# orybkin/video-gcp

Measured on AMD Instinct MI355X. Metric: predicted frames/sec, 64x64x3 seq_len=80 gcp_tree (posterior forward + all loss terms, model(inputs) and model.loss() of train.py:157-159, batch-stat BatchNorm), higher is better.
Workload: dtype f32 (encoder / decoder convs and the tree GEMMs from 512 rows: split-f16 MFMA with f32 accumulate, f32-equivalent; everything else exact f32 MFMA)

## Files before the change

### video-gcp_amd/csrc/conv3x3_lowres.hip

```cpp
#include "common.h"
#include "split_mfma.h"

namespace {

template <int CT, int HIN, int NCHUNK, int FPU>
struct LowresCfg {
    static constexpr int NW = 3 * CT, NT = NW * 64;
    static constexpr int NPIX = HIN * HIN, UPIX = FPU * NPIX, NPG = UPIX / 16, WOUT = 2 * HIN, HOUT = 2 * HIN;
    static constexpr int COUT = CT * 16, CIN = NCHUNK * 32, C4 = COUT / 4, Q4 = CIN / 4;
    static constexpr int YS = COUT + 4;
    static constexpr int PLANE_BYTES = UPIX * 64;
    static constexpr int PLANES_BYTES = NCHUNK * 2 * PLANE_BYTES;
    static constexpr int Y_BYTES = 9 * UPIX * YS * 4;
    static constexpr int Z_BYTES = FPU * 3 * HIN * WOUT * COUT * 4;
    static constexpr int PZ_BYTES = PLANES_BYTES > Z_BYTES ? PLANES_BYTES : Z_BYTES;
    static constexpr int TAB_BYTES = (2 * CIN + COUT) * 4;
    static constexpr int STAT_BYTES = NT * 8 * 4;
    static constexpr int LDS_BYTES = PZ_BYTES + Y_BYTES + 64 + TAB_BYTES + STAT_BYTES;
    static constexpr int NSLOT = UPIX * Q4;
    static constexpr int NS = (NSLOT + NT - 1) / NT;
    static constexpr int NHZ = FPU * 3 * HIN * WOUT * C4;
    static constexpr int NOUT = FPU * HOUT * WOUT * C4;
    static constexpr int NO = (NOUT + NT - 1) / NT;
    static_assert(NT % C4 == 0 && NT % Q4 == 0, "a thread keeps one channel quad of the input and one of the output");
    static_assert(NOUT * 16 <= Y_BYTES, "the finished output waits in the Y buffer");
    static_assert(LDS_BYTES <= 160 * 1024, "LDS");
};

__device__ __forceinline__ void up_taps(const int h, const int n, int& s0, int& s1, float& w0, float& w1) {
    const int s = h >> 1;
    const bool odd = h & 1;
    s0 = odd ? s : max(s - 1, 0);
    s1 = odd ? min(s + 1, n - 1) : s;
    w0 = odd ? 0.75f : 0.25f;
    w1 = 1.f - w0;
}

template <int CT, int HIN, int NCHUNK, int FPU>
__global__ void __launch_bounds__(3 * CT * 64, 1) conv3x3_lowres_kernel(const gcpx_conv_args a, const int stat_rows) {
    using Cfg = LowresCfg<CT, HIN, NCHUNK, FPU>;
    constexpr int NT = Cfg::NT, NPIX = Cfg::NPIX, UPIX = Cfg::UPIX, NPG = Cfg::NPG, WOUT = Cfg::WOUT, HOUT = Cfg::HOUT, COUT = Cfg::COUT;
    constexpr int C4 = Cfg::C4, Q4 = Cfg::Q4, NS = Cfg::NS, NSLOT = Cfg::NSLOT, NO = Cfg::NO, NOUT = Cfg::NOUT, NHZ = Cfg::NHZ;
    constexpr int PLANE = Cfg::PLANE_BYTES, YS = Cfg::YS, FS = HOUT * WOUT * COUT;
    extern __shared__ float4 smem4[];
    char* planes = reinterpret_cast<char*>(smem4);
    float* Z = reinterpret_cast<float*>(smem4);
    float* Y = reinterpret_cast<float*>(planes + Cfg::PZ_BYTES);
    unsigned* smax = reinterpret_cast<unsigned*>(planes + Cfg::PZ_BYTES + Cfg::Y_BYTES);
    float* bnS = reinterpret_cast<float*>(smax + 16);
    float* bnT = bnS + Cfg::CIN;
    float* biasT = bnT + Cfg::CIN;
    float4* stat = reinterpret_cast<float4*>(biasT + COUT);

    const int tid = threadIdx.x, lane = tid & 63;
    const int wave = __builtin_amdgcn_readfirstlane(tid >> 6);
    const int j = lane & 15, q = lane >> 4;
    const int tx = wave % 3, ct = wave / 3;
    const int F = a.F;
    const int ew = a.w_split_log2_dev ? __builtin_amdgcn_readfirstlane(*a.w_split_log2_dev) : a.w_split_log2;

    h8 wreg[3][NCHUNK][2];
    {
        const char* wbase = reinterpret_cast<const char*>(a.wpk_split) + lane * 16;
#pragma unroll
        for (int ty = 0; ty < 3; ++ty)
#pragma unroll
            for (int ch = 0; ch < NCHUNK; ++ch) {
                const char* wp = wbase + (size_t)(((ch * 9 + ty * 3 + tx) * CT + ct) * 2048);
                wreg[ty][ch][0] = *reinterpret_cast<const h8*>(wp);
                wreg[ty][ch][1] = *reinterpret_cast<const h8*>(wp + 1024);
            }
    }
    if (tid < NCHUNK) smax[tid] = 0u;

    const int cgq = (tid % Q4) * 4, chq = cgq >> 5;
    const int c0 = a.src[0].C;
    const bool first = cgq < c0;
    const int clq = first ? cgq : cgq - c0;
    const float* sptr = (first ? a.src[0].ptr : a.src[1].ptr) + clq;
    const int srcC = first ? a.src[0].C : a.src[1].C;
    const int fdiv = first ? a.src[0].frame_div : a.src[1].frame_div;
    const float slope = (first ? a.src[0].act : a.src[1].act) == GCPX_ACT_LRELU ? 0.2f : 1.f;
    const int c4q = tid % C4;
    for (int c = tid; c < Cfg::CIN; c += NT) {
        const gcpx_conv_src& sr = c < c0 ? a.src[0] : a.src[1];
        const int cl = c < c0 ? c : c - c0;
        bnS[c] = sr.scale ? sr.scale[cl] : 1.f;
        bnT[c] = sr.scale ? sr.shift[cl] : 0.f;
    }
    if (tid < COUT) biasT[tid] = a.bias[tid];
    stat[tid * 2] = stat[tid * 2 + 1] = make_float4(0.f, 0.f, 0.f, 0.f);

    float4 pre[NS];
    auto issue_loads = [&](const int f0, const int t) {
#pragma unroll
        for (int k = 0; k < NS; ++k) {
            const int idx = t + NT * k;
            pre[k] = make_float4(0.f, 0.f, 0.f, 0.f);
            if (NSLOT % NT == 0 || idx < NSLOT) {
                const int up = idx / Q4;
                const int f = min(f0 + up / NPIX, F - 1);
                pre[k] = *reinterpret_cast<const float4*>(sptr + ((size_t)(f / fdiv) * NPIX + up % NPIX) * srcC);
            }
        }
    };
    float4* O = reinterpret_cast<float4*>(Y);
    int pf0 = -1;
    auto store_out = [&](const int t) __attribute__((always_inline)) {
        float* outu = a.out + (size_t)pf0 * FS;
#pragma unroll
        for (int k = 0; k < NO; ++k) {
            const int i = t + NT * k;
            if ((NOUT % NT == 0 || i < NOUT) && pf0 + i / (HOUT * WOUT * C4) < F) *reinterpret_cast<float4*>(outu + i * 4) = O[i];
        }
    };

    const int nunits = (F + FPU - 1) / FPU;
    int u = blockIdx.x;
    if (u < nunits) issue_loads(u * FPU, tid);
    __syncthreads();

    for (; u < nunits; u += gridDim.x) {
        const int f0 = u * FPU;
        int tl = tid;
        asm volatile("" : "+v"(tl));
        float4 v[NS];
        float m = 0.f;
        const float4 bn_s = *reinterpret_cast<const float4*>(bnS + cgq), bn_t = *reinterpret_cast<const float4*>(bnT + cgq);
#pragma unroll
        for (int k = 0; k < NS; ++k) {
            float4 t = pre[k];
            t.x = fmaf(t.x, bn_s.x, bn_t.x); t.y = fmaf(t.y, bn_s.y, bn_t.y); t.z = fmaf(t.z, bn_s.z, bn_t.z); t.w = fmaf(t.w, bn_s.w, bn_t.w);
            t.x = t.x > 0.f ? t.x : t.x * slope; t.y = t.y > 0.f ? t.y : t.y * slope;
            t.z = t.z > 0.f ? t.z : t.z * slope; t.w = t.w > 0.f ? t.w : t.w * slope;
            if (!(NSLOT % NT == 0 || tl + NT * k < NSLOT)) t = make_float4(0.f, 0.f, 0.f, 0.f);
            v[k] = t;
            m = fmaxf(m, fmaxf(fmaxf(fabsf(t.x), fabsf(t.y)), fmaxf(fabsf(t.z), fabsf(t.w))));
        }
        m = fmaxf(m, __shfl_xor(m, 1));
        m = fmaxf(m, __shfl_xor(m, 2));
        m = fmaxf(m, __shfl_xor(m, 4));
        if ((lane & 7) == 0) atomicMax(&smax[chq], __float_as_uint(m));
        if (pf0 >= 0) store_out(tl);
        __syncthreads();
        int exr[NCHUNK];
#pragma unroll
        for (int ch = 0; ch < NCHUNK; ++ch) {
            const float amax = __uint_as_float(smax[ch]);
            int ec = 14 + 127 - (int)((__float_as_uint(amax) >> 23) & 0xff);
            ec = __builtin_amdgcn_readfirstlane(amax > 0.f ? max(-100, min(min(100, 126 - ew), ec)) : min(100, 126 - ew));
            exr[ch] = ch == 0 ? ec : min(ec, exr[ch - 1]);
        }
        {
            int ex = exr[0];
#pragma unroll
            for (int c = 1; c < NCHUNK; ++c) ex = chq == c ? exr[c] : ex;
            const float sc = __uint_as_float((unsigned)(127 + ex) << 23);
#pragma unroll
            for (int k = 0; k < NS; ++k) {
                const int idx = tl + NT * k;
                if (NSLOT % NT == 0 || idx < NSLOT) {
                    float4 s = v[k];
                    s.x *= sc; s.y *= sc; s.z *= sc; s.w *= sc;
                    h4 p1, p2;
                    p1[0] = (_Float16)s.x; p1[1] = (_Float16)s.y; p1[2] = (_Float16)s.z; p1[3] = (_Float16)s.w;
                    p2[0] = (_Float16)(s.x - (float)p1[0]); p2[1] = (_Float16)(s.y - (float)p1[1]);
                    p2[2] = (_Float16)(s.z - (float)p1[2]); p2[3] = (_Float16)(s.w - (float)p1[3]);
                    char* dst = planes + chq * 2 * PLANE + (idx / Q4) * 64 + (cgq & 31) * 2;
                    *reinterpret_cast<h4*>(dst) = p1;
                    *reinterpret_cast<h4*>(dst + PLANE) = p2;
                }
            }
        }
        __syncthreads();
        if (tid < NCHUNK) smax[tid] = 0u;
        if (u + (int)gridDim.x < nunits) issue_loads((u + gridDim.x) * FPU, tl);

        f32x4 acc[3][NPG];
#pragma unroll
        for (int ty = 0; ty < 3; ++ty)
#pragma unroll
            for (int pg = 0; pg < NPG; ++pg) acc[ty][pg] = f32x4{0, 0, 0, 0};
        __builtin_amdgcn_s_setprio(1);
#pragma unroll
        for (int ch = 0; ch < NCHUNK; ++ch) {
            if (ch > 0 && exr[ch] != exr[ch - 1]) {
                const float r = __uint_as_float((unsigned)(127 + exr[ch] - exr[ch - 1]) << 23);
#pragma unroll
                for (int ty = 0; ty < 3; ++ty)
#pragma unroll
                    for (int pg = 0; pg < NPG; ++pg) acc[ty][pg] *= r;
            }
#pragma unroll
            for (int pg = 0; pg < NPG; ++pg) {
                const char* bp = planes + ch * 2 * PLANE + (pg * 16 + (tl & 15)) * 64 + ((tl >> 4) & 3) * 16;
                const h8 b1 = *reinterpret_cast<const h8*>(bp);
                const h8 b2 = *reinterpret_cast<const h8*>(bp + PLANE);
#pragma unroll
                for (int ty = 0; ty < 3; ++ty) acc[ty][pg] = mfma32h(wreg[ty][ch][1], b1, acc[ty][pg]);
#pragma unroll
                for (int ty = 0; ty < 3; ++ty) acc[ty][pg] = mfma32h(wreg[ty][ch][0], b2, acc[ty][pg]);
#pragma unroll
                for (int ty = 0; ty < 3; ++ty) acc[ty][pg] = mfma32h(wreg[ty][ch][0], b1, acc[ty][pg]);
            }
        }
        __builtin_amdgcn_s_setprio(0);
        {
            const float inv = __uint_as_float((unsigned)(127 - exr[NCHUNK - 1] - ew) << 23);
#pragma unroll
            for (int ty = 0; ty < 3; ++ty)
#pragma unroll
                for (int pg = 0; pg < NPG; ++pg) {
                    const f32x4 y = acc[ty][pg] * inv;
                    *reinterpret_cast<float4*>(Y + ((ty * 3 + tx) * UPIX + pg * 16 + (tl & 15)) * YS + ct * 16 + ((tl >> 4) & 3) * 4) = make_float4(y[0], y[1], y[2], y[3]);
                }
        }
        __syncthreads();
        int tv = tid;
        asm volatile("" : "+v"(tv));
        float4 ab[NO];
#pragma unroll
        for (int k = 0; k < NO; ++k) ab[k] = *reinterpret_cast<const float4*>(biasT + c4q * 4);
        if (a.addend) {
#pragma unroll
            for (int k = 0; k < NO; ++k) {
                const int i = tv + NT * k;
                if (NOUT % NT == 0 || i < NOUT) {
                    const int f = min(f0 + i / (HOUT * WOUT * C4), F - 1);
                    const float4 ad = *reinterpret_cast<const float4*>(a.addend + (size_t)(f / a.addend_frame_div) * FS + (i % (HOUT * WOUT * C4)) * 4);
                    ab[k].x += ad.x; ab[k].y += ad.y; ab[k].z += ad.z; ab[k].w += ad.w;
                }
            }
        }

#pragma unroll 1
        for (int i = tv; i < NHZ; i += NT) {
            int t = i / C4;
            const int px = t % WOUT; t /= WOUT;
            const int sy = t % HIN; t /= HIN;
            const int ty = t % 3, fl = t / 3;
            float4 z = make_float4(0.f, 0.f, 0.f, 0.f);
#pragma unroll
            for (int kx = 0; kx < 3; ++kx) {
                const int hx = px + kx - 1;
                if (hx >= 0 && hx < WOUT) {
                    int s0, s1; float w0, w1;
                    up_taps(hx, HIN, s0, s1, w0, w1);
                    const float* yp = Y + ((ty * 3 + kx) * UPIX + fl * NPIX + sy * HIN) * YS + c4q * 4;
                    const float4 A = *reinterpret_cast<const float4*>(yp + s0 * YS);
                    const float4 B = *reinterpret_cast<const float4*>(yp + s1 * YS);
                    z.x += w0 * A.x + w1 * B.x; z.y += w0 * A.y + w1 * B.y; z.z += w0 * A.z + w1 * B.z; z.w += w0 * A.w + w1 * B.w;
                }
            }
            *reinterpret_cast<float4*>(Z + i * 4) = z;
        }
        __syncthreads();

        f32x4 st1 = f32x4{0, 0, 0, 0}, st2 = f32x4{0, 0, 0, 0};
#pragma unroll
        for (int k = 0; k < NO; ++k) {
            const int i = tv + NT * k;
            __builtin_amdgcn_sched_barrier(0);
            if (NOUT % NT == 0 || i < NOUT) {
                int t = i / C4;
                const int px = t % WOUT; t /= WOUT;
                const int py = t % HOUT, fl = t / HOUT;
                float4 o = make_float4(0.f, 0.f, 0.f, 0.f);
#pragma unroll
                for (int ky = 0; ky < 3; ++ky) {
                    const int hy = py + ky - 1;
                    if (hy >= 0 && hy < HOUT) {
                        int s0, s1; float w0, w1;
                        up_taps(hy, HIN, s0, s1, w0, w1);
                        const float* zp = Z + (((fl * 3 + ky) * HIN) * WOUT + px) * COUT + c4q * 4;
                        const float4 A = *reinterpret_cast<const float4*>(zp + s0 * WOUT * COUT);
                        const float4 B = *reinterpret_cast<const float4*>(zp + s1 * WOUT * COUT);
                        o.x += w0 * A.x + w1 * B.x; o.y += w0 * A.y + w1 * B.y; o.z += w0 * A.z + w1 * B.z; o.w += w0 * A.w + w1 * B.w;
                    }
                }
                const f32x4 r = f32x4{o.x + ab[k].x, o.y + ab[k].y, o.z + ab[k].z, o.w + ab[k].w};
                O[i] = make_float4(r[0], r[1], r[2], r[3]);
                if (f0 + fl < F) {
                    st1 += r;
                    st2 += r * r;
                }
            }
        }
        {
            const float4 s1 = stat[tid * 2], s2 = stat[tid * 2 + 1];
            stat[tid * 2] = make_float4(s1.x + st1[0], s1.y + st1[1], s1.z + st1[2], s1.w + st1[3]);
            stat[tid * 2 + 1] = make_float4(s2.x + st2[0], s2.y + st2[1], s2.z + st2[2], s2.w + st2[3]);
        }
        pf0 = f0;
    }
    if (pf0 >= 0) store_out(tid);

    if (a.stats_partial) {
        __syncthreads();
        const float* red = reinterpret_cast<const float*>(stat);
        if (tid < 2 * COUT) {
            const int which = tid / COUT, c = tid % COUT;
            float sum = 0.f;
#pragma unroll 4
            for (int m = 0; m < NT / C4; ++m) sum += red[((c >> 2) + C4 * m) * 8 + which * 4 + (c & 3)];
            a.stats_partial[((size_t)blockIdx.x * 2 + which) * COUT + c] = sum;
            for (int r = blockIdx.x + gridDim.x; r < stat_rows; r += gridDim.x) a.stats_partial[((size_t)r * 2 + which) * COUT + c] = 0.f;
        }
    }
}

template <int CT, int HIN, int NCHUNK, int FPU>
int launch_lowres(const gcpx_conv_args* a, hipStream_t stream, int rows) {
    using Cfg = LowresCfg<CT, HIN, NCHUNK, FPU>;
    auto kern = conv3x3_lowres_kernel<CT, HIN, NCHUNK, FPU>;
    static bool attr_set = false;
    if (!attr_set) {
        hipError_t e = hipFuncSetAttribute(reinterpret_cast<const void*>(kern), hipFuncAttributeMaxDynamicSharedMemorySize, Cfg::LDS_BYTES);
        if (e != hipSuccess) {
            gcpx_set_error("conv3x3 lowres: hipFuncSetAttribute(%d B LDS): %s", Cfg::LDS_BYTES, hipGetErrorString(e));
            return GCPX_ERR_HIP;
        }
        attr_set = true;
    }
    const int nunits = (a->F + FPU - 1) / FPU;
    int grid = gcpx_conv_grid() / 2;
    if (a->stats_partial && grid > rows) grid = rows;
    if (grid > nunits) grid = nunits;
    hipLaunchKernelGGL(kern, dim3(grid), dim3(Cfg::NT), Cfg::LDS_BYTES, stream, *a, rows);
    GCPX_CHECK_LAUNCH();
    return GCPX_OK;
}

int lowres_variant(const gcpx_conv_args* a) {
    if (!a || !a->upsample || !a->wpk_split || !a->out || !a->bias) return -1;
    if (a->split_layout != GCPX_SPLIT_PLAIN && a->split_layout != GCPX_SPLIT_LOWRES) return -1;
    if (a->head_mode != GCPX_HEAD_RAW || a->out_act != GCPX_ACT_NONE || a->out_pitch != a->Cout) return -1;
    if (a->src_row_map || a->raw_row_map || a->bwd_r) return -1;
    if (a->Hin != a->Win || a->Hout != 2 * a->Hin || a->Wout != 2 * a->Win || a->F <= 0) return -1;
    if (a->nsrc != 1 && a->nsrc != 2) return -1;
    int cin = 0;
    for (int s = 0; s < a->nsrc; ++s) {
        if (!a->src[s].ptr || a->src[s].C <= 0 || a->src[s].C % 16 || a->src[s].frame_div <= 0) return -1;
        cin += a->src[s].C;
    }
    if (cin != a->Cin) return -1;
    if (a->addend && a->addend_frame_div <= 0) return -1;
    if (a->Cout == 64 && a->Hin == 4 && a->Cin == 128) return 0;
    if (a->Cout == 32 && a->Hin == 8 && a->Cin == 64) return 1;
    if (a->Cout == 32 && a->Hin == 8 && a->Cin == 128) return 2;
    if (a->Cout == 32 && a->Hin == 4 && a->Cin == 128) return 3;
    return -1;
}

}

extern "C" int gcpx_conv3x3_lowres_supported(const gcpx_conv_args* a) { return lowres_variant(a) >= 0 ? 1 : 0; }

int gcpx_launch_lowres(const gcpx_conv_args* a, hipStream_t stream, int rows) {
    switch (lowres_variant(a)) {
        case 0: return launch_lowres<4, 4, 4, 2>(a, stream, rows);
        case 1: return launch_lowres<2, 8, 2, 1>(a, stream, rows);
        case 2: return launch_lowres<2, 8, 4, 1>(a, stream, rows);
        case 3: return launch_lowres<2, 4, 4, 2>(a, stream, rows);
    }
    gcpx_set_error("conv3x3 lowres: GCPX_SPLIT_LOWRES on a problem gcpx_conv3x3_lowres_supported refuses (up=%d Cin=%d Cout=%d Hin=%d)",
                   a->upsample, a->Cin, a->Cout, a->Hin);
    return GCPX_ERR_UNSUPPORTED;
}
```

### video-gcp_amd/weights.py

```python
import ctypes as C
import os
from contextlib import contextmanager

import torch

from . import packing as pk
from . import runtime as rt
from .hparams import GCPHParams
from .params import init_params, encoder_layers, encoder_skip_layers, decoder_layers
from .plan_ops import _addr


class WeightsMixin:

    def _flatten_params(self, params):
        off, self._poff = 0, {}
        for k, v in params.items():
            self._poff[k] = (off, tuple(v.shape))
            off += (v.numel() + 3) // 4 * 4
        self.theta = torch.zeros(off, dtype=torch.float32, device=self.device)
        self.sd = {}
        for k, v in params.items():
            o, shp = self._poff[k]
            view = self.theta[o:o + v.numel()].view(shp)
            view.copy_(v)
            self.sd[k] = view

    def _pack_predictor(self, prefix, out_dim):
        sd = self._psd
        mid = sd[f"{prefix}.input.linear.weight"].shape[0]
        n_mid = 0
        while f"{prefix}.pyramid-{n_mid}.linear.weight" in sd:
            n_mid += 1
        out_pad = (out_dim + 15) // 16 * 16
        w_in = sd[f"{prefix}.input.linear.weight"]
        k_raw = w_in.shape[1]
        if k_raw % 16:
            w_in = torch.cat([w_in, torch.zeros((mid, -k_raw % 16), dtype=w_in.dtype, device=w_in.device)], 1)
        d = dict(mid=mid, n_mid=n_mid, out_dim=out_dim, in_dim=w_in.shape[1], in_dim_raw=k_raw)
        d["w_in"] = pk.pack_gemm(w_in)
        d["b_in"] = sd[f"{prefix}.input.linear.bias"].contiguous()
        if n_mid:
            d["w_mid"] = torch.stack([pk.pack_gemm(sd[f"{prefix}.pyramid-{i}.linear.weight"]) for i in range(n_mid)]).contiguous()
            d["b_mid"] = torch.stack([sd[f"{prefix}.pyramid-{i}.linear.bias"] for i in range(n_mid)]).contiguous()
            d["gn_g"] = torch.stack([sd[f"{prefix}.pyramid-{i}.norm.weight"] for i in range(n_mid)]).contiguous()
            d["gn_b"] = torch.stack([sd[f"{prefix}.pyramid-{i}.norm.bias"] for i in range(n_mid)]).contiguous()
        d["w_out"] = pk.pack_gemm(sd[f"{prefix}.head.linear.weight"])
        d["b_out"] = pk.pad_vec(sd[f"{prefix}.head.linear.bias"], out_pad)
        return d

    def _pack_all(self):
        if self._arena is not None:
            self.repack()
            return
        self.pk = self._pack_tree(self.sd)
        if self._hp.tree_lstm:
            self._pack_fused_embed()
        self._pack_split()
        self._pack_gemm_split()

    def _pack_split(self):
        self.pk_split = {}
        hp = self._hp
        todo = []
        if hp.decoder_distribution == "discrete_logistic_mixture":
            todo.append(("dec.head", "decoder.gen_head.conv.weight", pk.dlm_channel_perm(hp.n_mixtures)))
            if self.head32 and hp.n_mixtures == 10 and hp.head_channels == 100:
                todo.append(("dec.head32", "decoder.gen_head.conv.weight", ("head32", pk.dlm_channel_perm(hp.n_mixtures))))
        hoist16 = set()
        for name, c_prev, c_skip, skip_idx, cout in decoder_layers(hp):
            if cout == 16 and c_prev + c_skip == 32:
                todo.append((f"dec.{name}", f"decoder.net.{name}.conv.weight", "rowfold"))
                if self.split_f16 and skip_idx >= 0 and c_prev == 16 and c_skip == 16 and os.environ.get("GCPX_NO_SKIP_HOIST") is None:
                    hoist16.add(f"dec.{name}")
            elif cout == 16:
                todo.append((f"dec.{name}", f"decoder.net.{name}.conv.weight", None))
            elif cout in (32, 64) and (c_prev + c_skip) % 32 == 0:
                todo.append((f"dec.{name}", f"decoder.net.{name}.conv.weight", "tiled32"))
        for name, cin, cout, norm in self._enc_layers[1:]:
            if cin == 16 or cin % 32 == 0:
                todo.append((f"enc.{name}", f"encoder.net.{name}.conv.weight", "enc4x4"))
        for name, key, perm in todo:
            off, shp = self._poff[key]
            d = {}
            if perm == "enc4x4":
                idx = pk.conv4x4_split_index(shp, off).to(self.device)
            elif perm == "rowfold":
                d["fold"] = torch.zeros(24 * shp[0] * shp[1], dtype=torch.float32, device=self.device)
                d["fold_src"] = (off, shp[0], shp[1])
                idx = pk.conv3x3_fold_index().to(self.device)
            elif perm == "tiled32":
                idx = pk.conv3x3_split32_index(shp, off).to(self.device)
            elif isinstance(perm, tuple) and perm[0] == "head32":
                idx = pk.head32_index(shp, off, perm[1]).to(self.device)
            else:
                idx = pk.conv3x3_split_index(shp, off, perm).to(self.device)
            d.update(idx=idx, out=torch.zeros(2 * idx.numel(), dtype=torch.int16, device=self.device),
                     log2=torch.zeros(1, dtype=torch.int32, device=self.device))
            self.pk_split[name] = d
            if perm == "rowfold" and name in hoist16:
                for tag, cbase in (("f16a", 0), ("f16b", 16)):
                    i16 = pk.conv3x3_fold16_index(shp[1], cbase).to(self.device)
                    self.pk_split[f"{name}.{tag}"] = dict(fold=d["fold"], fold16=True, idx=i16,
                                                          out=torch.zeros(2 * i16.numel(), dtype=torch.int16, device=self.device),
                                                          log2=torch.zeros(1, dtype=torch.int32, device=self.device))
        self.repack_split()

    def repack_split(self, stream=None):
        st = stream if stream is not None else torch.cuda.current_stream(self.device).cuda_stream
        if not self.pk_split:
            return
        tab = self._split_tab
        key = (self.theta.data_ptr(),) + tuple((d["out"].data_ptr(), d["idx"].data_ptr()) for d in self.pk_split.values())
        if tab is None or tab[2] != key:
            descs = []
            for name, d in self.pk_split.items():
                src = d["fold"] if "fold" in d else self.theta
                e = rt.SplitPackDesc()
                e.src, e.idx, e.out, e.log2_out, e.n = src.data_ptr(), d["idx"].data_ptr(), d["out"].data_ptr(), d["log2"].data_ptr(), d["idx"].numel()
                descs.append(e)
            arr = (rt.SplitPackDesc * len(descs))(*descs)
            dev = torch.frombuffer(bytearray(bytes(arr)), dtype=torch.uint8).to(self.device)
            tab = self._split_tab = (dev, len(descs), key, torch.zeros(len(descs), dtype=torch.int32, device=self.device))
        for name, d in self.pk_split.items():
            if "fold_src" in d:
                off, cout, cin = d["fold_src"]
                rt.check(self.lib.gcpx_fold_upsample_weights(self.theta.data_ptr() + 4 * off, cout, cin, d["fold"].data_ptr(), st), "fold_upsample_weights")
        rt.check(self.lib.gcpx_split_pack_group2(tab[0].data_ptr(), tab[1], tab[3].data_ptr(), st), "split_pack_group2")

    def _pack_gemm_split(self):
        self._gsplit = {}
        self._merge_side_rows = int(os.environ.get("GCPX_MERGE_SIDE_ROWS", "512")) or (1 << 60)
        pr = int(os.environ.get("GCPX_GEMM_PLANES_ROWS", "512"))
        self._planes_min_rows = pr if pr > 0 else 1 << 60
        if not self.split_f16:
            return
        for name, W in self.pk.items():
            if not (isinstance(W, dict) and name.startswith("tree")):
                continue
            for key, wpk in W.items():
                if not (key.endswith(".w") and (key.startswith("lstm") or key == "proj.w")):
                    continue
                stack = wpk if wpk.dim() == 5 else wpk[None]
                if (stack.shape[2] * 16) % 64 or (stack.shape[1] * 16) % 64:
                    continue
                packs = [pk.pack_gemm_split(pk.unpack_gemm(w, w.shape[1] * 16)) for w in stack]
                ws = torch.stack([p_[0] for p_ in packs]).contiguous().to(self.device)
                es = torch.tensor([p_[1] for p_ in packs], dtype=torch.int32, device=self.device)
                self._gsplit[wpk.data_ptr()] = (ws, es)

    def _set_split(self, a, name):
        d = self.pk_split.get(name)
        layout = None
        if name == "dec.head" and self.head32 and a.head_mode in (rt.HEAD_DLM_MEAN, rt.HEAD_DLM_NLL, rt.HEAD_DLM_NLL_GRAD) \
                and "dec.head32" in self.pk_split:
            d, layout = self.pk_split["dec.head32"], rt.SPLIT_HEAD32
        if self.split_f16 and d is not None:
            a.wpk_split, a.w_split_log2_dev = d["out"].data_ptr(), d["log2"].data_ptr()
            if layout is None:
                layout = rt.SPLIT_ROWFOLD16 if d.get("fold16") else (rt.SPLIT_ROWFOLD if "fold" in d else rt.SPLIT_PLAIN)
            a.split_layout = layout
            if layout == rt.SPLIT_PLAIN and os.environ.get("GCPX_NO_LOWRES") is None and \
                    (a.Cout == 64 or a.F <= self.lib.gcpx_conv_grid() // 2) and self.lib.gcpx_conv3x3_lowres_supported(C.byref(a)):
                a.split_layout = rt.SPLIT_LOWRES

    def _pack_fused_embed(self):
        hp = self._hp
        for l in range(hp.hierarchy_levels if hp.untied_layers else 1):
            p = f"tree_module.tree_modules.{l}.subgoal_pred"
            sd = self.sd
            We, be = sd[f"{p}.embed.weight"].double(), sd[f"{p}.embed.bias"].double()
            Wih = sd[f"{p}.lstm.0.weight_ih"].double()
            Wf = (Wih @ We).float()
            bf = (Wih @ be).float() + sd[f"{p}.lstm.0.bias_ih"]
            w, b = pk.lstm_gate_interleave(Wf, sd[f"{p}.lstm.0.weight_hh"], bf, sd[f"{p}.lstm.0.bias_hh"])
            self.pk[f"tree{l}"]["lstm0f.w"], self.pk[f"tree{l}"]["lstm0f.b"] = pk.pack_gemm(w), b

    def _pack_tree(self, sd):
        hp = self._hp
        self._psd = sd
        P = {}
        layers, c_top = encoder_layers(hp)
        self._enc_layers, self._c_top = layers, c_top
        P["enc.input.w"] = pk.pack_conv4x4_image(sd["encoder.net.input.conv.weight"])
        P["enc.input.b"] = sd["encoder.net.input.conv.bias"].contiguous()
        for name, cin, cout, norm in layers[1:]:
            P[f"enc.{name}.w"] = pk.pack_conv4x4(sd[f"encoder.net.{name}.conv.weight"])
            P[f"enc.{name}.b"] = sd[f"encoder.net.{name}.conv.bias"].contiguous()
        wh = sd["encoder.net.head.weight"]
        P["enc.head.w"] = pk.pack_gemm(wh.permute(0, 2, 3, 1).reshape(hp.nz_enc, 16 * c_top))
        P["enc.head.b"] = sd["encoder.net.head.bias"].contiguous()
        wt = sd["decoder.net.input.conv.weight"]
        P["dec.input.w"] = pk.pack_gemm(wt.permute(2, 3, 1, 0).reshape(16 * c_top, hp.nz_enc))
        P["dec.input.b"] = sd["decoder.net.input.conv.bias"].repeat(16).contiguous()
        for name, c_prev, c_skip, skip_idx, cout in decoder_layers(hp):
            P[f"dec.{name}.w"] = pk.pack_conv3x3(sd[f"decoder.net.{name}.conv.weight"], 16 if cout == 16 else 32)
            P[f"dec.{name}.b"] = pk.pad_vec(sd[f"decoder.net.{name}.conv.bias"], (cout + 15) // 16 * 16)
        hw, hb = sd["decoder.gen_head.conv.weight"], sd["decoder.gen_head.conv.bias"]
        if hp.decoder_distribution == "discrete_logistic_mixture":
            perm = pk.dlm_channel_perm(hp.n_mixtures)
            self._dlm_perm = torch.tensor(perm, device=self.device)
            P["dec.head.w"] = pk.pack_dlm_head(hw, perm)
            bk = torch.zeros(len(perm), device=hb.device, dtype=hb.dtype)
            permd = self._dlm_perm.to(hb.device)
            valid = permd >= 0
            bk[valid] = hb[permd[valid]]
            P["dec.head.b"] = bk
            self._head_pitch = len(perm)
        else:
            P["dec.head.w"] = pk.pack_conv3x3(hw, 16)
            P["dec.head.b"] = pk.pad_vec(hb, 16)
            self._head_pitch = 16
        seq_encs = [("seq", "inf_encoder")] + ([("kseq", "inf_key_encoder.0")] if hp.attentive_inference else [])
        if hp.seq_enc == "none":
            seq_encs = []
        for tag, pre in seq_encs:
            for nm in ["input"] + [f"pyramid-{i}" for i in range(hp.conv_inf_enc_layers)] + ["head"]:
                w = sd[f"{pre}.net.{nm}.conv.weight"]
                P[f"{tag}.{nm}.w"] = pk.pack_gemm(w.permute(0, 2, 1).reshape(w.shape[0], -1))
                P[f"{tag}.{nm}.b"] = sd[f"{pre}.net.{nm}.conv.bias"].contiguous()
        if hp.attentive_inference:
            P["kseq.key.w"] = pk.pack_gemm(sd["inf_key_encoder.1.linear.weight"])
            P["kseq.key.b"] = sd["inf_key_encoder.1.linear.bias"].contiguous()
        if hp.regress_length:
            P["length_pred"] = self._pack_predictor("length_pred.p", hp.max_seq_len)
        if hp.attach_state_regressor:
            P["state_regressor"] = self._pack_predictor("state_regressor", hp.state_dim)
        if hp.attach_inv_mdl:
            P["inv_mdl"] = self._pack_predictor("inv_mdl.action_pred", hp.n_actions)
        if hp.attach_cost_mdl:
            P["cost_mdl"] = self._pack_predictor("cost_mdl.cost_pred", 1)
        self._pack_latent_model(P)
        return P

    def build_arena(self, extra_pack=None):
        dev = self.device
        def probe(only_hh):
            sd = {}
            for k, (o, shp) in self._poff.items():
                n = 1
                for d in shp:
                    n *= d
                hh = k.endswith("bias_hh")
                if hh == only_hh:
                    sd[k] = (torch.arange(n, device=dev, dtype=torch.float64) + (o + 1)).view(shp)
                else:
                    sd[k] = torch.zeros(shp, device=dev, dtype=torch.float64)
            P = self._pack_tree(sd)
            X = extra_pack(sd) if extra_pack is not None else {}
            return P, X
        (P0, X0), (P1, X1) = probe(False), probe(True)
        leaves = []
        def walk(d0, d1, path):
            for k in d0:
                if isinstance(d0[k], dict):
                    walk(d0[k], d1[k], path + (k,))
                elif torch.is_tensor(d0[k]):
                    leaves.append((path + (k,), d0, d0[k], d1[k]))
        walk(P0, P1, ("P",))
        walk(X0, X1, ("X",))
        from .dist import gradient_bucket_ranges
        ranges = gradient_bucket_ranges(self._poff, self._hp.hierarchy_levels, self._hp.untied_layers)
        rest = len(ranges) - 1
        def bucket_of(t0, t1):
            ids = torch.cat([t0.reshape(-1), t1.reshape(-1)])
            ids = ids[ids > 0] - 1
            if ids.numel() == 0:
                return rest
            lo, hi = int(ids.min()), int(ids.max())
            for i, (_, a, b) in enumerate(ranges):
                if a <= lo and hi < b:
                    return i
            return rest
        leaves = [lf + (bucket_of(lf[2], lf[3]),) for lf in leaves]
        leaves.sort(key=lambda lf: (bool((lf[3] > 0).any()), lf[4]))
        leaves = [lf[:4] + (lf[4],) for lf in leaves]
        total = sum((lf[2].numel() + 3) // 4 * 4 for lf in leaves)
        self._arena = torch.zeros(total, dtype=torch.float32, device=dev)
        idx0 = torch.full((total,), -1, dtype=torch.int32, device=dev)
        idx1 = torch.full((total,), -1, dtype=torch.int32, device=dev)
        off = 0
        self._arena_split = None
        runs = {}
        for path, holder, t0, t1, bkt in leaves:
            n = t0.numel()
            two = bool((t1 > 0).any())
            if self._arena_split is None and two:
                self._arena_split = off
            idx0[off:off + n] = (t0.reshape(-1) - 1).to(torch.int32)
            idx1[off:off + n] = (t1.reshape(-1) - 1).to(torch.int32)
            holder[path[-1]] = self._arena[off:off + n].view(t0.shape)
            r = runs.setdefault((bkt, two), [off, off])
            assert r[1] == off, "leaves of one slice are contiguous inside a half"
            off += (n + 3) // 4 * 4
            r[1] = off
        self._arena_runs = {ranges[b][0]: [] for b in range(len(ranges))}
        for (bkt, two), (a, b) in sorted(runs.items()):
            self._arena_runs[ranges[bkt][0]].append((a, b - a, two))
        self._arena_ranges = ranges
        self._arena_idx0, self._arena_idx1 = idx0, idx1
        self._psd = self.sd
        self.pk = P0
        self._extra_packs = X0
        self._clear_plans()
        self.repack()
        return X0

    def repack(self, stream=None, bucket=None, max_blocks=0):
        st = stream if stream is not None else torch.cuda.current_stream(self.device).cuda_stream
        self._enc_frames_pack = None
        if bucket is not None:
            for off, cnt, two in self._arena_runs[bucket]:
                rt.check(self.lib.gcpx_repack_blocks(self.theta.data_ptr(), self._arena_idx0.data_ptr() + 4 * off,
                                                     (self._arena_idx1.data_ptr() + 4 * off) if two else None, self._arena.data_ptr() + 4 * off,
                                                     cnt, max_blocks, st), "repack")
            self._repack_gsplit(st, bucket)
            if bucket == self._arena_ranges[-1][0]:
                self.repack_split(st)
            return
        n, sp = self._arena.numel(), self._arena_split
        sp = n if sp is None else sp
        if sp > 0:
            rt.check(self.lib.gcpx_repack(self.theta.data_ptr(), self._arena_idx0.data_ptr(), None, self._arena.data_ptr(), sp, st), "repack")
        if sp < n:
            rt.check(self.lib.gcpx_repack(self.theta.data_ptr(), self._arena_idx0.data_ptr() + 4 * sp, self._arena_idx1.data_ptr() + 4 * sp,
                                          self._arena.data_ptr() + 4 * sp, n - sp, st), "repack")
        self._repack_gsplit(st, None)
        self.repack_split(st)

    def _repack_gsplit(self, st, bucket):
        for name, (tab, n, scratch) in self._gsplit_tabs.items():
            if bucket is None or bucket == name:
                rt.check(self.lib.gcpx_split_pack_group2(tab.data_ptr(), n, scratch.data_ptr(), st), "split_pack_group2")

    def _pack_hsp(self, prefix, n_layers):
        sd, T = self._psd, {}
        T["embed.w"] = pk.pack_gemm(sd[f"{prefix}.embed.weight"])
        T["embed.b"] = sd[f"{prefix}.embed.bias"].contiguous()
        for i in range(n_layers):
            w, b = pk.lstm_gate_interleave(sd[f"{prefix}.lstm.{i}.weight_ih"], sd[f"{prefix}.lstm.{i}.weight_hh"],
                                           sd[f"{prefix}.lstm.{i}.bias_ih"], sd[f"{prefix}.lstm.{i}.bias_hh"])
            T[f"lstm{i}.w"], T[f"lstm{i}.b"] = pk.pack_gemm(w), b
        T["out.w"] = pk.pack_gemm(sd[f"{prefix}.out.weight"])
        T["out.b"] = sd[f"{prefix}.out.bias"].contiguous()
        return T

    def _pack_latent_model(self, P):
        hp, sd = self._hp, self._psd
        if hp.adaptive:
            P["distance"] = self._pack_predictor("tree_module.tree_modules.0.binding.distance_predictor", 1)
        else:
            P["existence"] = self._pack_predictor("tree_module.tree_modules.0.binding.existence_predictor", 1)
        H = hp.nz_mid_lstm
        n_mod = hp.hierarchy_levels if hp.untied_layers else 1
        if hp.attentive_inference:
            att = lambda l, nm: sd[f"tree_module.tree_modules.{l}.inference.attention.attention_layers.0.{nm}"]
            for nm in ("k_proj", "v_proj"):
                P[f"attn.{nm}.w"] = torch.stack([pk.pack_gemm(att(l, f"{nm}.weight")) for l in range(n_mod)]).contiguous()
                P[f"attn.{nm}.b"] = torch.stack([att(l, f"{nm}.bias") for l in range(n_mod)]).contiguous()
        for l in range(hp.hierarchy_levels if hp.untied_layers else 1):
            p = f"tree_module.tree_modules.{l}"
            T = {}
            T["prior"] = self._pack_predictor(f"{p}.prior", 2 * hp.nz_vae)
            T["q"] = self._pack_predictor(f"{p}.inference.q", 2 * hp.nz_vae)
            if not hp.tree_lstm:
                T["sg"] = self._pack_predictor(f"{p}.subgoal_pred.net", hp.nz_enc)
                P[f"tree{l}"] = T
                if hp.attentive_inference:
                    raise ValueError("attentive inference with the non-LSTM subgoal predictor is not built")
                continue
            T["embed.w"] = pk.pack_gemm(sd[f"{p}.subgoal_pred.embed.weight"])
            T["embed.b"] = sd[f"{p}.subgoal_pred.embed.bias"].contiguous()
            for i in range(hp.n_lstm_layers):
                w, b = pk.lstm_gate_interleave(sd[f"{p}.subgoal_pred.lstm.{i}.weight_ih"], sd[f"{p}.subgoal_pred.lstm.{i}.weight_hh"],
                                               sd[f"{p}.subgoal_pred.lstm.{i}.bias_ih"], sd[f"{p}.subgoal_pred.lstm.{i}.bias_hh"])
                T[f"lstm{i}.w"], T[f"lstm{i}.b"] = pk.pack_gemm(w), b
            T["out.w"] = pk.pack_gemm(sd[f"{p}.subgoal_pred.out.weight"])
            T["out.b"] = sd[f"{p}.subgoal_pred.out.bias"].contiguous()
            nproj = 2 * hp.n_lstm_layers
            if hp.tree_lstm == "split_linear":
                T["proj.w"] = torch.stack([pk.pack_gemm(sd[f"{p}.subgoal_pred.projections.{j}.weight"]) for j in range(nproj)]).contiguous()
                T["proj.b"] = torch.stack([sd[f"{p}.subgoal_pred.projections.{j}.bias"] for j in range(nproj)]).contiguous()
            elif hp.tree_lstm == "linear":
                T["proj.w"] = pk.pack_gemm(sd[f"{p}.subgoal_pred.projection.weight"])
                T["proj.b"] = sd[f"{p}.subgoal_pred.projection.bias"].contiguous()
            if l == 0 and hp.lstm_init == "mlp":
                T["init"] = self._pack_predictor(f"{p}.lstm_initializer.net", 2 * hp.lstm_state_dim)
            if hp.attentive_inference:
                a = f"{p}.inference.attention"
                T["attn.query"] = self._pack_predictor(f"{a}.query_net", hp.nz_attn_key)
                for nm, key in (("q_proj", f"{a}.attention_layers.0.q_proj"), ("out_proj", f"{a}.attention_layers.0.out_proj"),
                                ("out", f"{a}.out")):
                    T[f"attn.{nm}.w"] = pk.pack_gemm(sd[f"{key}.weight"])
                    T[f"attn.{nm}.b"] = sd[f"{key}.bias"].contiguous()
            P[f"tree{l}"] = T
```

Before: 518,800.

## Restructure lowres conv upsample epilogue into per-thread half-runs with register reuse

Rewrites the bilinear-upsample epilogue of the low-resolution 3x3 conv kernel so each thread handles one half-run of output rows along a column or row. The source taps are loaded once into registers and reused across neighbouring outputs instead of being reloaded from LDS per pixel. When registers allow, results and the bias/addend are kept in registers rather than staged in LDS. It also replaces shuffles with ds_swizzle for the max reduction, hoists per-frame source index math, and enables the lowres path for all supported shapes instead of only small-frame or 64-channel cases. The wider gating may route shapes to this kernel where it underperforms, and the added register pressure risks spills.

```diff
diff --git a/video-gcp_amd/csrc/conv3x3_lowres.hip b/video-gcp_amd/csrc/conv3x3_lowres.hip
--- a/video-gcp_amd/csrc/conv3x3_lowres.hip
+++ b/video-gcp_amd/csrc/conv3x3_lowres.hip
@@ -19,11 +19,11 @@
     static constexpr int LDS_BYTES = PZ_BYTES + Y_BYTES + 64 + TAB_BYTES + STAT_BYTES;
     static constexpr int NSLOT = UPIX * Q4;
     static constexpr int NS = (NSLOT + NT - 1) / NT;
-    static constexpr int NHZ = FPU * 3 * HIN * WOUT * C4;
-    static constexpr int NOUT = FPU * HOUT * WOUT * C4;
-    static constexpr int NO = (NOUT + NT - 1) / NT;
+    static constexpr int NH = 2 * FPU * 3 * HIN * C4;
+    static constexpr int NV = 2 * FPU * WOUT * C4;
     static_assert(NT % C4 == 0 && NT % Q4 == 0, "a thread keeps one channel quad of the input and one of the output");
-    static_assert(NOUT * 16 <= Y_BYTES, "the finished output waits in the Y buffer");
+    static_assert(NH == NT && NV <= NT && NV % 64 == 0, "one horizontal half-run per thread; whole wavefronts in the vertical stage");
+    static_assert(NV * HIN * 16 <= Y_BYTES, "a finished unit may wait in the Y buffer");
     static_assert(LDS_BYTES <= 160 * 1024, "LDS");
 };
 
@@ -36,12 +36,43 @@
     w1 = 1.f - w0;
 }
 
+template <int HIN, bool TAPWISE>
+__device__ __forceinline__ void half_run(const float* const (&p)[3], const int ss, float4 (&o)[HIN]) {
+    constexpr int NS1 = HIN / 2 + 1;
+    int dep = 0;
+#pragma unroll
+    for (int k = 0; k < 3; ++k) {
+        if (TAPWISE && k > 0) {
+#pragma unroll
+            for (int r = k > 1 ? 0 : 1; r < HIN; ++r) asm volatile("" : "+v"(dep) : "v"(o[r].x), "v"(o[r].w));
+        }
+        const float* pk = p[k] + dep;
+        float4 L[NS1];
+#pragma unroll
+        for (int s = 0; s < NS1; ++s)
+            if (k > 0 || s < NS1 - 1) L[s] = *reinterpret_cast<const float4*>(pk + s * ss);
+#pragma unroll
+        for (int r = 0; r < HIN; ++r) {
+            const int h = r + k - 1;
+            if (h >= 0) {
+                int s0, s1; float w0, w1;
+                up_taps(h, HIN, s0, s1, w0, w1);
+                const float4 A = L[s0], B = L[s1];
+                const float4 t = make_float4(w0 * A.x + w1 * B.x, w0 * A.y + w1 * B.y, w0 * A.z + w1 * B.z, w0 * A.w + w1 * B.w);
+                if (k == 0 || (k == 1 && r == 0)) o[r] = t;
+                else { o[r].x += t.x; o[r].y += t.y; o[r].z += t.z; o[r].w += t.w; }
+            }
+        }
+    }
+}
+
 template <int CT, int HIN, int NCHUNK, int FPU>
 __global__ void __launch_bounds__(3 * CT * 64, 1) conv3x3_lowres_kernel(const gcpx_conv_args a, const int stat_rows) {
     using Cfg = LowresCfg<CT, HIN, NCHUNK, FPU>;
     constexpr int NT = Cfg::NT, NPIX = Cfg::NPIX, UPIX = Cfg::UPIX, NPG = Cfg::NPG, WOUT = Cfg::WOUT, HOUT = Cfg::HOUT, COUT = Cfg::COUT;
-    constexpr int C4 = Cfg::C4, Q4 = Cfg::Q4, NS = Cfg::NS, NSLOT = Cfg::NSLOT, NO = Cfg::NO, NOUT = Cfg::NOUT, NHZ = Cfg::NHZ;
+    constexpr int C4 = Cfg::C4, Q4 = Cfg::Q4, NS = Cfg::NS, NSLOT = Cfg::NSLOT, NV = Cfg::NV;
     constexpr int PLANE = Cfg::PLANE_BYTES, YS = Cfg::YS, FS = HOUT * WOUT * COUT;
+    constexpr bool REG_RICH = CT * NCHUNK <= 4, AB_EARLY = REG_RICH;
     extern __shared__ float4 smem4[];
     char* planes = reinterpret_cast<char*>(smem4);
     float* Z = reinterpret_cast<float*>(smem4);
@@ -73,15 +104,7 @@
     }
     if (tid < NCHUNK) smax[tid] = 0u;
 
-    const int cgq = (tid % Q4) * 4, chq = cgq >> 5;
     const int c0 = a.src[0].C;
-    const bool first = cgq < c0;
-    const int clq = first ? cgq : cgq - c0;
-    const float* sptr = (first ? a.src[0].ptr : a.src[1].ptr) + clq;
-    const int srcC = first ? a.src[0].C : a.src[1].C;
-    const int fdiv = first ? a.src[0].frame_div : a.src[1].frame_div;
-    const float slope = (first ? a.src[0].act : a.src[1].act) == GCPX_ACT_LRELU ? 0.2f : 1.f;
-    const int c4q = tid % C4;
     for (int c = tid; c < Cfg::CIN; c += NT) {
         const gcpx_conv_src& sr = c < c0 ? a.src[0] : a.src[1];
         const int cl = c < c0 ? c : c - c0;
@@ -93,25 +116,42 @@
 
     float4 pre[NS];
     auto issue_loads = [&](const int f0, const int t) {
+        const int cgq = (t % Q4) * 4;
+        const bool first = cgq < c0;
+        const float* sptr = (first ? a.src[0].ptr : a.src[1].ptr) + (first ? cgq : cgq - c0);
+        const int srcC = first ? a.src[0].C : a.src[1].C;
+        int sf[FPU];
+#pragma unroll
+        for (int fl = 0; fl < FPU; ++fl) {
+            const int f = min(f0 + fl, F - 1);
+            const int q0 = f / a.src[0].frame_div, q1 = a.nsrc > 1 ? f / a.src[1].frame_div : 0;
+            sf[fl] = first ? q0 : q1;
+        }
 #pragma unroll
         for (int k = 0; k < NS; ++k) {
             const int idx = t + NT * k;
             pre[k] = make_float4(0.f, 0.f, 0.f, 0.f);
             if (NSLOT % NT == 0 || idx < NSLOT) {
                 const int up = idx / Q4;
-                const int f = min(f0 + up / NPIX, F - 1);
-                pre[k] = *reinterpret_cast<const float4*>(sptr + ((size_t)(f / fdiv) * NPIX + up % NPIX) * srcC);
+                int fs = sf[0];
+#pragma unroll
+                for (int fl = 1; fl < FPU; ++fl) fs = up / NPIX == fl ? sf[fl] : fs;
+                pre[k] = *reinterpret_cast<const float4*>(sptr + ((size_t)fs * NPIX + up % NPIX) * srcC);
             }
         }
     };
+    float4 keep[HIN];
     float4* O = reinterpret_cast<float4*>(Y);
     int pf0 = -1;
     auto store_out = [&](const int t) __attribute__((always_inline)) {
-        float* outu = a.out + (size_t)pf0 * FS;
-#pragma unroll
-        for (int k = 0; k < NO; ++k) {
-            const int i = t + NT * k;
-            if ((NOUT % NT == 0 || i < NOUT) && pf0 + i / (HOUT * WOUT * C4) < F) *reinterpret_cast<float4*>(outu + i * 4) = O[i];
+        if (t < NV) {
+            const int px = (t / C4) % WOUT, fl = (t / (C4 * WOUT)) % FPU, hv = t / (C4 * WOUT * FPU);
+            if (pf0 + fl < F) {
+                float* op = a.out + (size_t)(pf0 + fl) * FS + ((hv ? HOUT - 1 : 0) * WOUT + px) * COUT + (t % C4) * 4;
+                const int os = hv ? -WOUT * COUT : WOUT * COUT;
+#pragma unroll
+                for (int r = 0; r < HIN; ++r) *reinterpret_cast<float4*>(op + r * os) = REG_RICH ? keep[r] : O[r * NV + t];
+            }
         }
     };
 
@@ -124,6 +164,8 @@
         const int f0 = u * FPU;
         int tl = tid;
         asm volatile("" : "+v"(tl));
+        const int cgq = (tl % Q4) * 4, chq = cgq >> 5;
+        const float slope = (cgq < c0 ? a.src[0].act : a.src[1].act) == GCPX_ACT_LRELU ? 0.2f : 1.f;
         float4 v[NS];
         float m = 0.f;
         const float4 bn_s = *reinterpret_cast<const float4*>(bnS + cgq), bn_t = *reinterpret_cast<const float4*>(bnT + cgq);
@@ -137,9 +179,9 @@
             v[k] = t;
             m = fmaxf(m, fmaxf(fmaxf(fabsf(t.x), fabsf(t.y)), fmaxf(fabsf(t.z), fabsf(t.w))));
         }
-        m = fmaxf(m, __shfl_xor(m, 1));
-        m = fmaxf(m, __shfl_xor(m, 2));
-        m = fmaxf(m, __shfl_xor(m, 4));
+        m = fmaxf(m, __int_as_float(__builtin_amdgcn_ds_swizzle(__float_as_int(m), 0x041f)));
+        m = fmaxf(m, __int_as_float(__builtin_amdgcn_ds_swizzle(__float_as_int(m), 0x081f)));
+        m = fmaxf(m, __int_as_float(__builtin_amdgcn_ds_swizzle(__float_as_int(m), 0x101f)));
         if ((lane & 7) == 0) atomicMax(&smax[chq], __float_as_uint(m));
         if (pf0 >= 0) store_out(tl);
         __syncthreads();
@@ -173,8 +215,38 @@
             }
         }
         __syncthreads();
-        if (tid < NCHUNK) smax[tid] = 0u;
-        if (u + (int)gridDim.x < nunits) issue_loads((u + gridDim.x) * FPU, tl);
+        if (tl < NCHUNK) smax[tl] = 0u;
+        auto addend_frame = [&](const int fl) __attribute__((always_inline)) {
+            int q = 0;
+            if (a.addend) {
+#pragma unroll
+                for (int g = 0; g < FPU; ++g) {
+                    const int qg = min(f0 + g, F - 1) / a.addend_frame_div;
+                    q = fl == g ? qg : q;
+                }
+            }
+            return q;
+        };
+        float4 ab[HIN];
+        auto issue_addend = [&](const int t) __attribute__((always_inline)) {
+            if (t < NV) {
+                const float4 bq = *reinterpret_cast<const float4*>(biasT + (t % C4) * 4);
+#pragma unroll
+                for (int r = 0; r < HIN; ++r) ab[r] = bq;
+                if (a.addend) {
+                    const int px = (t / C4) % WOUT, fl = (t / (C4 * WOUT)) % FPU, hv = t / (C4 * WOUT * FPU);
+                    const float* ap = a.addend + (size_t)addend_frame(fl) * FS + ((hv ? HOUT - 1 : 0) * WOUT + px) * COUT + (t % C4) * 4;
+                    const int os = hv ? -WOUT * COUT : WOUT * COUT;
+#pragma unroll
+                    for (int r = 0; r < HIN; ++r) {
+                        const float4 ad = *reinterpret_cast<const float4*>(ap + r * os);
+                        ab[r].x += ad.x; ab[r].y += ad.y; ab[r].z += ad.z; ab[r].w += ad.w;
+                    }
+                }
+            }
+        };
+        if (AB_EARLY) issue_addend(tl);
+        issue_loads((u + (int)gridDim.x < nunits ? u + (int)gridDim.x : u) * FPU, tl);
 
         f32x4 acc[3][NPG];
 #pragma unroll
@@ -218,78 +290,57 @@
         __syncthreads();
         int tv = tid;
         asm volatile("" : "+v"(tv));
-        float4 ab[NO];
-#pragma unroll
-        for (int k = 0; k < NO; ++k) ab[k] = *reinterpret_cast<const float4*>(biasT + c4q * 4);
-        if (a.addend) {
-#pragma unroll
-            for (int k = 0; k < NO; ++k) {
-                const int i = tv + NT * k;
-                if (NOUT % NT == 0 || i < NOUT) {
-                    const int f = min(f0 + i / (HOUT * WOUT * C4), F - 1);
-                    const float4 ad = *reinterpret_cast<const float4*>(a.addend + (size_t)(f / a.addend_frame_div) * FS + (i % (HOUT * WOUT * C4)) * 4);
-                    ab[k].x += ad.x; ab[k].y += ad.y; ab[k].z += ad.z; ab[k].w += ad.w;
+        const int c4o = (tv % C4) * 4;
+
+        {
+            int t = tv / C4;
+            const int sy = t % HIN; t /= HIN;
+            const int ty = t % 3; t /= 3;
+            const int fl = t % FPU, h = t / FPU;
+            const float* yb = Y + ((ty * 3 + (h ? 2 : 0)) * UPIX + fl * NPIX + sy * HIN + (h ? HIN - 1 : 0)) * YS + c4o;
+            const int ts = h ? -UPIX * YS : UPIX * YS;
+            const float* const yp[3] = {yb, yb + ts, yb + 2 * ts};
+            float4 z[HIN];
+            half_run<HIN, !REG_RICH>(yp, h ? -YS : YS, z);
+            float* zp = Z + (((fl * 3 + ty) * HIN + sy) * WOUT + (h ? WOUT - 1 : 0)) * COUT + c4o;
+            const int zs = h ? -COUT : COUT;
+#pragma unroll
+            for (int r = 0; r < HIN; ++r) *reinterpret_cast<float4*>(zp + r * zs) = z[r];
+        }
+        __syncthreads();
+
+        if (tv < NV) {
+            int t = tv / C4;
+            const int px = t % WOUT; t /= WOUT;
+            const int fl = t % FPU, hv = t / FPU;
+            const float* zb = Z + (((fl * 3 + (hv ? 2 : 0)) * HIN + (hv ? HIN - 1 : 0)) * WOUT + px) * COUT + c4o;
+            const int ts = hv ? -HIN * WOUT * COUT : HIN * WOUT * COUT;
+            const float* const zq[3] = {zb, zb + ts, zb + 2 * ts};
+            float4 o[HIN];
+            half_run<HIN, !REG_RICH>(zq, hv ? -WOUT * COUT : WOUT * COUT, o);
+            const float4 bq = *reinterpret_cast<const float4*>(biasT + c4o);
+            const float* ap = a.addend + (size_t)addend_frame(fl) * FS + ((hv ? HOUT - 1 : 0) * WOUT + px) * COUT + c4o;
+            const int os = hv ? -WOUT * COUT : WOUT * COUT;
+            f32x4 st1, st2;
+#pragma unroll
+            for (int r = 0; r < HIN; ++r) {
+                float4 b = AB_EARLY ? ab[r] : bq;
+                if (!AB_EARLY && a.addend) {
+                    __builtin_amdgcn_sched_barrier(0);
+                    const float4 ad = *reinterpret_cast<const float4*>(ap + r * os);
+                    b.x += ad.x; b.y += ad.y; b.z += ad.z; b.w += ad.w;
                 }
-            }
-        }
-
-#pragma unroll 1
-        for (int i = tv; i < NHZ; i += NT) {
-            int t = i / C4;
-            const int px = t % WOUT; t /= WOUT;
-            const int sy = t % HIN; t /= HIN;
-            const int ty = t % 3, fl = t / 3;
-            float4 z = make_float4(0.f, 0.f, 0.f, 0.f);
-#pragma unroll
-            for (int kx = 0; kx < 3; ++kx) {
-                const int hx = px + kx - 1;
-                if (hx >= 0 && hx < WOUT) {
-                    int s0, s1; float w0, w1;
-                    up_taps(hx, HIN, s0, s1, w0, w1);
-                    const float* yp = Y + ((ty * 3 + kx) * UPIX + fl * NPIX + sy * HIN) * YS + c4q * 4;
-                    const float4 A = *reinterpret_cast<const float4*>(yp + s0 * YS);
-                    const float4 B = *reinterpret_cast<const float4*>(yp + s1 * YS);
-                    z.x += w0 * A.x + w1 * B.x; z.y += w0 * A.y + w1 * B.y; z.z += w0 * A.z + w1 * B.z; z.w += w0 * A.w + w1 * B.w;
-                }
-            }
-            *reinterpret_cast<float4*>(Z + i * 4) = z;
-        }
-        __syncthreads();
-
-        f32x4 st1 = f32x4{0, 0, 0, 0}, st2 = f32x4{0, 0, 0, 0};
-#pragma unroll
-        for (int k = 0; k < NO; ++k) {
-            const int i = tv + NT * k;
-            __builtin_amdgcn_sched_barrier(0);
-            if (NOUT % NT == 0 || i < NOUT) {
-                int t = i / C4;
-                const int px = t % WOUT; t /= WOUT;
-                const int py = t % HOUT, fl = t / HOUT;
-                float4 o = make_float4(0.f, 0.f, 0.f, 0.f);
-#pragma unroll
-                for (int ky = 0; ky < 3; ++ky) {
-                    const int hy = py + ky - 1;
-                    if (hy >= 0 && hy < HOUT) {
-                        int s0, s1; float w0, w1;
-                        up_taps(hy, HIN, s0, s1, w0, w1);
-                        const float* zp = Z + (((fl * 3 + ky) * HIN) * WOUT + px) * COUT + c4q * 4;
-                        const float4 A = *reinterpret_cast<const float4*>(zp + s0 * WOUT * COUT);
-                        const float4 B = *reinterpret_cast<const float4*>(zp + s1 * WOUT * COUT);
-                        o.x += w0 * A.x + w1 * B.x; o.y += w0 * A.y + w1 * B.y; o.z += w0 * A.z + w1 * B.z; o.w += w0 * A.w + w1 * B.w;
-                    }
-                }
-                const f32x4 r = f32x4{o.x + ab[k].x, o.y + ab[k].y, o.z + ab[k].z, o.w + ab[k].w};
-                O[i] = make_float4(r[0], r[1], r[2], r[3]);
-                if (f0 + fl < F) {
-                    st1 += r;
-                    st2 += r * r;
-                }
-            }
-        }
-        {
-            const float4 s1 = stat[tid * 2], s2 = stat[tid * 2 + 1];
-            stat[tid * 2] = make_float4(s1.x + st1[0], s1.y + st1[1], s1.z + st1[2], s1.w + st1[3]);
-            stat[tid * 2 + 1] = make_float4(s2.x + st2[0], s2.y + st2[1], s2.z + st2[2], s2.w + st2[3]);
+                const f32x4 v4 = f32x4{o[r].x + b.x, o[r].y + b.y, o[r].z + b.z, o[r].w + b.w};
+                if (REG_RICH) keep[r] = make_float4(v4[0], v4[1], v4[2], v4[3]);
+                else O[r * NV + tv] = make_float4(v4[0], v4[1], v4[2], v4[3]);
+                st1 = r == 0 ? v4 : st1 + v4;
+                st2 = r == 0 ? v4 * v4 : st2 + v4 * v4;
+            }
+            if (f0 + fl < F) {
+                const float4 s1 = stat[tv * 2], s2 = stat[tv * 2 + 1];
+                stat[tv * 2] = make_float4(s1.x + st1[0], s1.y + st1[1], s1.z + st1[2], s1.w + st1[3]);
+                stat[tv * 2 + 1] = make_float4(s2.x + st2[0], s2.y + st2[1], s2.z + st2[2], s2.w + st2[3]);
+            }
         }
         pf0 = f0;
     }
diff --git a/video-gcp_amd/weights.py b/video-gcp_amd/weights.py
--- a/video-gcp_amd/weights.py
+++ b/video-gcp_amd/weights.py
@@ -161,7 +161,7 @@
                 layout = rt.SPLIT_ROWFOLD16 if d.get("fold16") else (rt.SPLIT_ROWFOLD if "fold" in d else rt.SPLIT_PLAIN)
             a.split_layout = layout
             if layout == rt.SPLIT_PLAIN and os.environ.get("GCPX_NO_LOWRES") is None and \
-                    (a.Cout == 64 or a.F <= self.lib.gcpx_conv_grid() // 2) and self.lib.gcpx_conv3x3_lowres_supported(C.byref(a)):
+                    self.lib.gcpx_conv3x3_lowres_supported(C.byref(a)):
                 a.split_layout = rt.SPLIT_LOWRES
 
     def _pack_fused_embed(self):
```

After: 531,200, median of 6. 2.4% higher.
